# Tanveer81/ReVisionLLM

Hardware: AMD Instinct MI355X
Metric: video-segments/sec (whole node), stage-2 100-seg recursion, Vicuna-7B (higher is better)
Workload: dtype fp16

## Files before the change

### revisionllm_amd/csrc/gemm_rows.hip

```cpp
#include <hip/hip_runtime.h>

#include <atomic>
#include <type_traits>

#include "kernels.h"
#include "gemv_finish.h"

#ifndef RS_PROBE
#define RS_PROBE 0
#endif
#ifndef RS_PART
#define RS_PART 0
#endif
#ifndef RS_DW_BIG
#define RS_DW_BIG 4
#endif

namespace {

typedef const __attribute__((address_space(1))) void* gptr_t;
typedef __attribute__((address_space(3))) void* lptr_t;
__device__ __forceinline__ void glds16(const void* g, void* l) { __builtin_amdgcn_global_load_lds((gptr_t)g, (lptr_t)l, 16, 0, 0); }

typedef unsigned int rs_u32x4 __attribute__((ext_vector_type(4)));
constexpr int RS_SC1 = 16;
__device__ __forceinline__ void st_sc1(__amdgpu_buffer_rsrc_t r, unsigned byte_off, f32x4 v) {
    __builtin_amdgcn_raw_buffer_store_b128(__builtin_bit_cast(rs_u32x4, v), r, (int)byte_off, 0, RS_SC1);
}
__device__ __forceinline__ f32x4 ld_sc1(__amdgpu_buffer_rsrc_t r, unsigned byte_off) {
    return __builtin_bit_cast(f32x4, __builtin_amdgcn_raw_buffer_load_b128(r, (int)byte_off, 0, RS_SC1));
}

constexpr int RS_W = 4;
constexpr int RS_THREADS = (RS_W + 1) * 64;
template <int MB, int WP = 1> struct RowsCfg {
    static constexpr int DW = WP == 2 ? 8 : (MB >= 8 ? RS_DW_BIG : 4), LPS = WP == 2 ? 2 : 4, DX = MB == 4 ? 4 : 3, WPE = MB <= 5 ? 3 : 2;
};
typedef unsigned int rs_w8 __attribute__((ext_vector_type(4)));

constexpr bool rows_sumsq_at_head(int MB) { return MB >= 8; }
template <int MB, int NTH, int PTB>
__device__ __forceinline__ void rows_sumsq(const GemvNorm& nrm, float* ssq, int tg) {
    if (!nrm.in_sumsq || (RS_PROBE & 16)) return;
    constexpr int CHAINS = MB * 128;
    constexpr int PT = (CHAINS + NTH - 1) / NTH;
    const int nblk = nrm.in_nblk;
    const int off = (RS_PROBE & 2048) ? 0 : (int)((blockIdx.x >> 3) * 37u) % CHAINS;
#pragma unroll
    for (int i0 = 0; i0 < PT; i0 += PTB) {
        f32x4 pj[PTB][8];
        int cc[PTB];
#pragma unroll
        for (int i = 0; i < PTB; ++i) {
            const int idx = tg + (i0 + i) * NTH;
            int c = idx + off;
            c = c >= CHAINS ? c - CHAINS : c;
            cc[i] = (i0 + i < PT && idx < CHAINS) ? c : -1;
            const int mb = c >> 7, q = (c >> 2) & 31, rq = c & 3;
            const float* src = nrm.in_sumsq + ((int64_t)(mb * nblk + q) * 16 + rq * 4);
#pragma unroll
            for (int j = 0; j < 8; ++j) {
                const bool have = q + 32 * j < nblk;
                const f32x4 v = *(const f32x4*)(src + (have ? j * 512 : 0));
                pj[i][j] = have ? v : f32x4{0.f, 0.f, 0.f, 0.f};
            }
        }
        __builtin_amdgcn_sched_barrier(0);
#pragma unroll
        for (int i = 0; i < PTB; ++i) {
            if (cc[i] < 0) continue;
            const int c = cc[i], mb = c >> 7, q = (c >> 2) & 31, rq = c & 3;
            f32x4 a = f32x4{0.f, 0.f, 0.f, 0.f};
#pragma unroll
            for (int j = 0; j < 8; ++j) a += pj[i][j];
            for (int b = q + 256; b < nblk; b += 32) a += *(const f32x4*)(nrm.in_sumsq + ((int64_t)(mb * nblk + b) * 16 + rq * 4));
            *(f32x4*)(ssq + mb * 512 + q * 16 + rq * 4) = a;
        }
    }
}

template <int MB>
__device__ __forceinline__ void rows_sumsq_total(const float* ssq, float* totl, int t) {
    if (t < MB * 16) {
        const int mb = t >> 4, row = t & 15;
        float tot = 0.f;
#pragma unroll
        for (int q = 0; q < 32; ++q) tot += ssq[(mb * 32 + q) * 16 + row];
        totl[t] = tot;
    }
}

template <int MB, int PPW, int PAIRS, int WP>
__device__ __forceinline__ void rows_qkv_finish(const f32x4 (&sres)[PPW], int wave, int cg, int fr, int kg, int M, const GemvNorm& nrm, const QkvRope& qr,
                                                const float* totl) {
    const int D = qr.H * 128;
    const int n0 = cg * 64;
    const int sec = n0 >= 2 * D ? 2 : n0 >= D ? 1 : 0;
    const int hd0 = n0 - sec * D, head = hd0 >> 7;
    int posv[PPW];
    f32x4 cf[PPW], wsc[PPW];
#pragma unroll
    for (int i = 0; i < PPW; ++i) {
        const int p = wave + RS_W * i < PAIRS ? wave + RS_W * i : PAIRS - 1;
        const int tile = p / MB, mb = p % MB, b = mb * 16 + fr;
        const int pc = (hd0 & 127) + tile * 16 + kg * 4;
        const int bc = b < M ? b : M - 1;
        posv[i] = b < M ? qr.row_pos[bc] : -1;
        cf[i] = sec < 2 ? *(const f32x4*)(qr.cs + ((int64_t)bc * 64 + (pc >> 1)) * 2) : f32x4{0.f, 0.f, 0.f, 0.f};
        if constexpr (WP == 2) wsc[i] = *(const f32x4*)(nrm.w_scale + n0 + tile * 16 + kg * 4);
    }
    __builtin_amdgcn_sched_barrier(0);
#pragma unroll
    for (int i = 0; i < PPW; ++i) {
        const int p = wave + RS_W * i;
        if (p >= PAIRS) break;
        const int tile = p / MB, mb = p % MB, b = mb * 16 + fr;
        const int pc = (hd0 & 127) + tile * 16 + kg * 4;
        f32x4 v = sres[i];
        if constexpr (WP == 2) v *= wsc[i];
        if (nrm.in_sumsq) v *= rsqrtf(__fmaf_rn(totl[mb * 16 + fr], nrm.inv_d, nrm.eps));
        const int pos = posv[i];
        if (pos < 0 || pos >= qr.Smax) continue;
        if (sec < 2) {
            const f32x4 t = cf[i];
            const float a0 = __fmaf_rn(v[0], t[0], -__fmul_rn(v[1], t[1])), b0 = __fmaf_rn(v[1], t[0], __fmul_rn(v[0], t[1]));
            const float a1 = __fmaf_rn(v[2], t[2], -__fmul_rn(v[3], t[3])), b1 = __fmaf_rn(v[3], t[2], __fmul_rn(v[2], t[3]));
            const u32x2 o = pack_op16x4(f32x4{a0, b0, a1, b1});
            if (sec == 0) *(u32x2*)((op16_t*)qr.q16 + (int64_t)b * D + hd0 + tile * 16 + kg * 4) = o;
            else *(u32x2*)((op16_t*)qr.kc + (((int64_t)b * qr.H + head) * qr.Smax + pos) * 128 + pc) = o;
        } else {
            op16_t* dst = (op16_t*)qr.vtc + ((int64_t)b * qr.H + head) * 128 * qr.Smax + rv_vt_index(pc, pos);
#pragma unroll
            for (int r = 0; r < 4; ++r) dst[r * 8] = f32_to_op16(v[r]);
        }
    }
}

#ifndef RS_PF_N
#define RS_PF_N 8
#endif
constexpr int RS_PF = RS_PF_N;
#ifndef RS_EARLY_READS
#define RS_EARLY_READS 0
#endif
constexpr bool rows_early(int MB) { return RS_EARLY_READS && MB >= 8 && !(RS_PROBE & (4 | 4096)); }
template <int MB, int WP>
__device__ __forceinline__ void rows_stage_schedule() {
#ifndef RS_NO_STAGE_SCHEDULE
    if constexpr (MB >= 8 && !(RS_PROBE & 4)) {
        constexpr int R = 4 * MB;
        if constexpr (!rows_early(MB)) __builtin_amdgcn_sched_group_barrier(0x100, RS_PF, 0);
#ifdef RS_EARLY_PIN_VMEM
        else __builtin_amdgcn_sched_group_barrier(0x020, WP == 2 ? 2 : 4, 0);
#endif
#pragma unroll
        for (int i = 0; i < R - RS_PF; ++i) {
            __builtin_amdgcn_sched_group_barrier(0x008, 1, 0);
            __builtin_amdgcn_sched_group_barrier(0x100, 1, 0);
        }
        __builtin_amdgcn_sched_group_barrier(0x008, RS_PF, 0);
    }
#endif
}

template <int MB, int VPW, int FIN, int WP = 1>
__global__ __attribute__((amdgpu_flat_work_group_size(RS_THREADS, RS_THREADS), amdgpu_waves_per_eu(RowsCfg<MB>::WPE, RowsCfg<MB>::WPE))) void
rows_kernel(const op16_t* __restrict__ X, const op16_t* __restrict__ W, float* __restrict__ planes, const float* __restrict__ bias,
            const float* res, int64_t ldr, void* Cv, int64_t ldc, int M, int N, int K, GemvNorm nrm, QkvRope qr) {
    extern __shared__ __attribute__((aligned(16))) char rs_smem[];
    constexpr int S = 8 / VPW, LOG = VPW == 8 ? 3 : VPW == 4 ? 2 : VPW == 2 ? 1 : 0;
    constexpr int DW = RowsCfg<MB, WP>::DW, DX = RowsCfg<MB, WP>::DX, LPS = RowsCfg<MB, WP>::LPS;
    constexpr int SLAB = MB * 4096;
    constexpr int XL = MB * 4;
    static_assert((DX - 2) * XL <= 63 && (DW - 2) * LPS <= 63, "vmcnt is a 6-bit counter");
    const int tid = threadIdx.x, lane = tid & 63;
    const int wave = __builtin_amdgcn_readfirstlane(tid >> 6);
    const int cg = blockIdx.x / S, sp = blockIdx.x % S;
    const int nkb = K >> 7;
    const int ntile = cg * RS_W + (wave < RS_W ? wave : 0);
    auto vcount = [&](int i) -> int { return (nkb - (sp * VPW + i) + 7) >> 3; };
    int T = 0;
#pragma unroll
    for (int i = 0; i < VPW; ++i) T += vcount(i);

    f32x4 acc[MB], stk[LOG ? LOG : 1][MB];
#pragma unroll
    for (int mb = 0; mb < MB; ++mb) acc[mb] = f32x4{0.f, 0.f, 0.f, 0.f};

    if (wave == RS_W) {
        int pi = 0, pc = 0;
        auto next_kb = [&]() -> int {
            int kb = -1;
            if (pi < VPW) {
                kb = sp * VPW + pi + 8 * pc;
                if (++pc == vcount(pi)) { pc = 0; ++pi; }
            }
            return kb;
        };
        auto issue = [&](int g) {
            const int kb = next_kb();
            const op16_t* xs = X + (kb >= 0 ? (int64_t)kb * (MB * 2048) : 0) + lane * 8;
            char* dst = rs_smem + (g % DX) * SLAB;
#pragma unroll
            for (int i = 0; i < XL; ++i) glds16(xs + i * 512, dst + i * 1024);
        };
        if constexpr (!(RS_PROBE & 8))
            for (int d = 0; d < DX - 1; ++d) issue(d);
        if constexpr (rows_sumsq_at_head(MB)) {
            if (nrm.in_sumsq && !(RS_PROBE & 16)) __builtin_amdgcn_s_barrier();
        }
        for (int g = 0; g < T; ++g) {
            asm volatile("s_waitcnt vmcnt(%0)" ::"n"((DX - 2) * XL) : "memory");
            if constexpr (!(RS_PROBE & 2)) __builtin_amdgcn_s_barrier();
            if constexpr (!(RS_PROBE & 8)) issue(g + DX - 1);
        }
        asm volatile("s_waitcnt vmcnt(0)" ::: "memory");
    } else {
        const op16_t* wp = W + (int64_t)ntile * (K >> 5) * (WP == 2 ? 256 : 512) + lane * 8;
        typename std::conditional<WP == 2, rs_w8, op16x8>::type wf[DW][LPS];
        int li = 0, lc = 0;
        int ci = 0, cc = 0;
#define RS_ISSUE_W(slot)                                                                                                             \
    do {                                                                                                                             \
        int kb_ = -1;                                                                                                                \
        if (li < VPW) {                                                                                                              \
            kb_ = sp * VPW + li + 8 * lc;                                                                                            \
            if (++lc == vcount(li)) { lc = 0; ++li; }                                                                                \
        }                                                                                                                            \
        const op16_t* ws_ = kb_ >= 0 ? ((RS_PROBE & 1) ? W + lane * 8 + (kb_ & 1) * 2048 : wp + (int64_t)((RS_PROBE & 8192) ? (kb_ + ((int)blockIdx.x * RS_W + wave) * 5) % nkb : kb_) * (WP == 2 ? 1024 : 2048)) : X + lane * 8; \
        _Pragma("unroll") for (int j_ = 0; j_ < LPS; ++j_)                                                                          \
            wf[slot][j_] = __builtin_nontemporal_load((const typename std::remove_reference<decltype(wf[0][0])>::type*)(ws_ + j_ * 512)); \
    } while (0)
#pragma unroll
        for (int d = 0; d < DW - 1; ++d) RS_ISSUE_W(d);
        if constexpr (rows_sumsq_at_head(MB)) {
            if (nrm.in_sumsq && !(RS_PROBE & 16)) {
                float* ssq_ = (float*)(rs_smem + DX * SLAB);
                rows_sumsq<MB, 256, 3>(nrm, ssq_, tid);
                asm volatile("s_waitcnt lgkmcnt(0)" ::: "memory");
                __builtin_amdgcn_s_barrier();
                rows_sumsq_total<MB>(ssq_, ssq_ + MB * 512, tid);
                asm volatile("s_waitcnt lgkmcnt(0)" ::: "memory");
            }
        }
        unsigned long long* stamps = (unsigned long long*)(rs_smem + DX * SLAB + MB * (2048 + 64));
        const bool stamping = (RS_PROBE & 16384) && S == 1 && wave == 0 && blockIdx.x == 8;
#define RS_STAMP(k_)                                                                       \
    if constexpr (RS_PROBE & 16384) {                                                      \
        if (stamping && g < 64) {                                                          \
            const unsigned long long t_ = __builtin_amdgcn_s_memtime();                    \
            if (lane == 0) stamps[g * 4 + (k_)] = t_;                                      \
        }                                                                                  \
    }
        if constexpr (RS_PROBE & 16384) {
            if (stamping) {
                for (int i = lane; i < 256; i += 64) stamps[i] = 0ull;
            }
        }
        for (int g0 = 0; g0 < T; g0 += DW) {
#pragma unroll
            for (int u = 0; u < DW; ++u) {
                const int g = g0 + u;
                if (g < T) {
                    RS_STAMP(0)
                    asm volatile("s_waitcnt vmcnt(%0)" ::"n"((DW - 2) * LPS) : "memory");
                    RS_STAMP(1)
                    if constexpr (!(RS_PROBE & 2)) __builtin_amdgcn_s_barrier();
                    RS_STAMP(2)
                    op16x8 pre[rows_early(MB) ? RS_PF : 1];
                    if constexpr (rows_early(MB)) {
                        const char* xs0 = rs_smem + (g % DX) * SLAB + lane * 16;
#pragma unroll
                        for (int i = 0; i < RS_PF; ++i) pre[i] = *(const op16x8*)(xs0 + i * 1024);
                    }
                    RS_ISSUE_W((u + DW - 1) % DW);
                    {
                        const char* xs = rs_smem + (g % DX) * SLAB + lane * 16;
#pragma unroll
                        for (int j = 0; j < 4; ++j) {
                            op16x8 wj;
                            if constexpr (WP == 2) wj = fp8x8_to_op16x8(wf[u][j >> 1][(j & 1) * 2], wf[u][j >> 1][(j & 1) * 2 + 1]);
                            else wj = wf[u][j];
#pragma unroll
                            for (int mb = 0; mb < MB; ++mb) {
                                const op16x8 xf = (rows_early(MB) && j * MB + mb < RS_PF) ? pre[(j * MB + mb) % RS_PF]
                                                                                           : *(const op16x8*)(xs + ((RS_PROBE & 4096) ? 0 : (j * MB + mb) * 1024));
                                if constexpr (RS_PROBE & 4) {
                                    if (mb == 0) acc[0][0] += __builtin_bit_cast(f32x4, wj)[j & 3] + __builtin_bit_cast(f32x4, xf)[0];
                                } else {
                                    acc[mb] = rv_mfma16(wj, xf, acc[mb]);
                                }
                            }
                        }
                        rows_stage_schedule<MB, WP>();
                    }
                    RS_STAMP(3)
                    if (++cc == vcount(ci)) {
                        if constexpr (VPW > 1) {
                            bool placed = false;
#pragma unroll
                            for (int b = 0; b < LOG; ++b) {
                                if (placed) continue;
                                if ((ci >> b) & 1) {
#pragma unroll
                                    for (int mb = 0; mb < MB; ++mb) acc[mb] = stk[b][mb] + acc[mb];
                                } else {
#pragma unroll
                                    for (int mb = 0; mb < MB; ++mb) stk[b][mb] = acc[mb];
                                    placed = true;
                                }
                            }
                            if (placed) {
#pragma unroll
                                for (int mb = 0; mb < MB; ++mb) acc[mb] = f32x4{0.f, 0.f, 0.f, 0.f};
                            }
                        }
                        cc = 0;
                        ++ci;
                    }
                }
            }
        }
#undef RS_ISSUE_W
#undef RS_STAMP
        if constexpr (RS_PROBE & 16384) {
            if (stamping) {
                asm volatile("s_waitcnt lgkmcnt(0)" ::: "memory");
                for (int i = lane; i < 256; i += 64) ((unsigned long long*)planes)[i] = stamps[i];
            }
        }
    }
    const unsigned plane = (unsigned)(N >> 4) * MB * 1024;
    const __amdgpu_buffer_rsrc_t pr = __builtin_amdgcn_make_buffer_rsrc(planes, 0, 0x7ffffff0, 0x00020000);
    constexpr int XCH_OFF = MB * 2048 > 16384 ? MB * 2048 : 16384;
    static_assert(XCH_OFF + RS_W * MB * 1024 <= DX * MB * 4096, "the exchange area must fit the slab ring");
    char* xch = rs_smem + XCH_OFF;
    if constexpr (S == 1) {
        asm volatile("s_waitcnt vmcnt(0)" ::: "memory");
        __syncthreads();
        if (wave < RS_W) {
#pragma unroll
            for (int mb = 0; mb < MB; ++mb) *(f32x4*)(xch + ((wave * MB + mb) * 64 + lane) * 16) = acc[mb];
        }
    } else {
        if (wave < RS_W) {
            const unsigned off = sp * plane + ((unsigned)ntile * MB * 64 + lane) * 16;
#pragma unroll
            for (int mb = 0; mb < MB; ++mb) st_sc1(pr, off + mb * 1024, acc[mb]);
        }
        asm volatile("s_waitcnt vmcnt(0)" ::: "memory");
    }
    __syncthreads();
    __shared__ int is_last;
    if constexpr (S > 1) {
        if (tid == 0) {
            unsigned* cnt = (unsigned*)nrm.arrive + (LOG * (RV_ROWS_COUNTERS / 4) + cg);
            is_last = __hip_atomic_fetch_add(cnt, 1u, __ATOMIC_RELAXED, __HIP_MEMORY_SCOPE_AGENT) % S == S - 1;
        }
        __syncthreads();
        if (!is_last) return;
    }
    constexpr int NT = (FIN == 1 || FIN == 2) ? 2 : 1;
    constexpr int OUT_BF16 = (FIN == 1 || FIN == 4) ? 1 : 0;
    constexpr int ACT = FIN == 1 ? RV_ACT_SILU_MUL : RV_ACT_NONE;
    constexpr int ROPE = FIN == 3 ? 1 : 0;
    constexpr int BPG = RS_W / NT;
    constexpr int PAIRS = BPG * MB;
    constexpr int PPW = (PAIRS + RS_W - 1) / RS_W;
    const int fr = lane & 15, kg = lane >> 4;
    const int nblk = N / (16 * NT);
    f32x4 pl[PPW][NT][S];
    if (wave < RS_W) {
#pragma unroll
        for (int i = 0; i < PPW; ++i) {
            const int p = wave + RS_W * i < PAIRS ? wave + RS_W * i : PAIRS - 1;
            const int blk = cg * BPG + p / MB, mb = p % MB;
#pragma unroll
            for (int t = 0; t < NT; ++t) {
                if constexpr (S == 1) {
                    pl[i][t][0] = *(const f32x4*)(xch + (((p / MB * NT + t) * MB + mb) * 64 + lane) * 16);
                } else {
                    const unsigned q = (((unsigned)(blk * NT + t) * MB + mb) * 64 + lane) * 16;
#pragma unroll
                    for (int w = 0; w < S; ++w) pl[i][t][w] = ld_sc1(pr, q + w * plane);
                }
            }
        }
    }
    float* ssq = (float*)(rs_smem + (rows_sumsq_at_head(MB) ? DX * SLAB : 0));
    if constexpr (!rows_sumsq_at_head(MB)) {
        if (nrm.in_sumsq && !(RS_PROBE & 16)) {
            rows_sumsq<MB, RS_THREADS, 2>(nrm, ssq, tid);
            __syncthreads();
            rows_sumsq_total<MB>(ssq, ssq + MB * 512, tid);
            __syncthreads();
        }
    }
    const float* totl = ssq + MB * 512;
    if (wave >= RS_W) return;
    if constexpr (ROPE) {
        if (qr.row_pos && qr.G == 1 && !(RS_PROBE & 64)) {
            f32x4 sv[PPW];
#pragma unroll
            for (int i = 0; i < PPW; ++i) {
                if constexpr (S == 8) sv[i] = gemv_tree8(pl[i][0]);
                else if constexpr (S == 4) sv[i] = (pl[i][0][0] + pl[i][0][1]) + (pl[i][0][2] + pl[i][0][3]);
                else if constexpr (S == 2) sv[i] = pl[i][0][0] + pl[i][0][1];
                else sv[i] = pl[i][0][0];
            }
            rows_qkv_finish<MB, PPW, PAIRS, WP>(sv, wave, cg, fr, kg, M, nrm, qr, totl);
            return;
        }
    }
#pragma unroll
    for (int i = 0; i < PPW; ++i) {
        const int p = wave + RS_W * i;
        if (p >= PAIRS) break;
        const int blk = cg * BPG + p / MB, mb = p % MB;
        f32x4 sres[NT];
#pragma unroll
        for (int t = 0; t < NT; ++t) {
            if constexpr (S == 8) sres[t] = gemv_tree8(pl[i][t]);
            else if constexpr (S == 4) sres[t] = (pl[i][t][0] + pl[i][t][1]) + (pl[i][t][2] + pl[i][t][3]);
            else if constexpr (S == 2) sres[t] = pl[i][t][0] + pl[i][t][1];
            else sres[t] = pl[i][t][0];
        }
        const float tot = nrm.in_sumsq ? totl[mb * 16 + fr] : 0.f;
        const f32x4 z = f32x4{0.f, 0.f, 0.f, 0.f};
        gemv_finish<NT, OUT_BF16, ACT, WP, ROPE>(sres, mb, fr, kg, blk, nblk, M, N, bias, res, ldr, Cv, ldc, nrm, qr, tot, z, z, z, z, false);
    }
}

constexpr int RS_MAXIT = 8;
template <int MB, int VPW, int FIN, int WP = 1>
__global__ __attribute__((amdgpu_flat_work_group_size(RS_THREADS, RS_THREADS), amdgpu_waves_per_eu(RowsCfg<MB>::WPE, RowsCfg<MB>::WPE))) void
rows_kernel_p(const op16_t* __restrict__ X, const op16_t* __restrict__ W, float* __restrict__ planes, const float* __restrict__ bias,
            const float* res, int64_t ldr, void* Cv, int64_t ldc, int M, int N, int K, GemvNorm nrm, QkvRope qr) {
    extern __shared__ __attribute__((aligned(16))) char rs_smem[];
    constexpr int S = 8 / VPW, LOG = VPW == 8 ? 3 : VPW == 4 ? 2 : VPW == 2 ? 1 : 0;
    constexpr int DW = RowsCfg<MB, WP>::DW, DX = RowsCfg<MB, WP>::DX, LPS = RowsCfg<MB, WP>::LPS;
    constexpr int SLAB = MB * 4096;
    constexpr int XL = MB * 4;
    static_assert((DX - 2) * XL <= 63 && (DW - 2) * LPS <= 63, "vmcnt is a 6-bit counter");
    const int tid = threadIdx.x, lane = tid & 63;
    const int wave = __builtin_amdgcn_readfirstlane(tid >> 6);
    const int nitems = (N >> 6) * S, G = (int)gridDim.x;
    const int sp = blockIdx.x % S;
    const int nkb = K >> 7;
    const int n_it = (nitems - (int)blockIdx.x + G - 1) / G;
    auto vcount = [&](int i) -> int { return (nkb - (sp * VPW + i) + 7) >> 3; };
    int T = 0;
#pragma unroll
    for (int i = 0; i < VPW; ++i) T += vcount(i);
    const int Tp = (T + DW - 1) / DW * DW;
    const unsigned plane = (unsigned)(N >> 4) * MB * 1024;
    const __amdgpu_buffer_rsrc_t pr = __builtin_amdgcn_make_buffer_rsrc(planes, 0, 0x7ffffff0, 0x00020000);

    f32x4 acc[MB], stk[LOG ? LOG : 1][MB];
#pragma unroll
    for (int mb = 0; mb < MB; ++mb) acc[mb] = f32x4{0.f, 0.f, 0.f, 0.f};

    if (wave == RS_W) {
        int pi = 0, pc = 0, pp = 0, pn = 0;
        auto issue = [&](int g) {
            int kb = -1;
            if (pn < n_it) {
                if (pp < T) {
                    kb = sp * VPW + pi + 8 * pc;
                    if (++pc == vcount(pi)) { pc = 0; ++pi; }
                }
                if (++pp == Tp) { pp = 0; pi = 0; ++pn; }
            }
            const op16_t* xs = X + (kb >= 0 ? (int64_t)kb * (MB * 2048) : 0) + lane * 8;
            char* dst = rs_smem + (g % DX) * SLAB;
#pragma unroll
            for (int i = 0; i < XL; ++i) glds16(xs + i * 512, dst + i * 1024);
        };
        if constexpr (!(RS_PROBE & 8))
            for (int d = 0; d < DX - 1; ++d) issue(d);
        if constexpr (rows_sumsq_at_head(MB)) {
            if (nrm.in_sumsq && !(RS_PROBE & 16)) __builtin_amdgcn_s_barrier();
        }
        const int TT = n_it * Tp;
        for (int g = 0; g < TT; ++g) {
            asm volatile("s_waitcnt vmcnt(%0)" ::"n"((DX - 2) * XL) : "memory");
            if constexpr (!(RS_PROBE & 2)) __builtin_amdgcn_s_barrier();
            if constexpr (!(RS_PROBE & 8)) issue(g + DX - 1);
        }
    } else {
        const int64_t tile_stride = (int64_t)(K >> 5) * (WP == 2 ? 256 : 512);
        const int64_t item_stride = (int64_t)(G / S) * RS_W * tile_stride;
        const op16_t* wp = W + ((int)blockIdx.x / S * RS_W + wave) * tile_stride + lane * 8;
        typename std::conditional<WP == 2, rs_w8, op16x8>::type wf[DW][LPS];
        int li = 0, lc = 0, lp = 0, ln = 0;
#define RS_ISSUE_W(slot)                                                                                                             \
    do {                                                                                                                             \
        const op16_t* ws_ = X + lane * 8;                                                                                            \
        if (ln < n_it) {                                                                                                             \
            if (lp < T) {                                                                                                            \
                const int kb_ = sp * VPW + li + 8 * lc;                                                                              \
                ws_ = (RS_PROBE & 1) ? W + lane * 8 + (kb_ & 1) * 2048 : wp + (int64_t)((RS_PROBE & 8192) ? (kb_ + ((int)blockIdx.x * RS_W + wave) * 5) % (K >> 7) : kb_) * (WP == 2 ? 1024 : 2048);                 \
                if (++lc == vcount(li)) { lc = 0; ++li; }                                                                            \
            }                                                                                                                        \
            if (++lp == Tp) { lp = 0; li = 0; ++ln; wp += item_stride; }                                                             \
        }                                                                                                                            \
        _Pragma("unroll") for (int j_ = 0; j_ < LPS; ++j_)                                                                          \
            wf[slot][j_] = __builtin_nontemporal_load((const typename std::remove_reference<decltype(wf[0][0])>::type*)(ws_ + j_ * 512)); \
    } while (0)
#pragma unroll
        for (int d = 0; d < DW - 1; ++d) RS_ISSUE_W(d);
        if constexpr (rows_sumsq_at_head(MB)) {
            if (nrm.in_sumsq && !(RS_PROBE & 16)) {
                float* ssq_ = (float*)(rs_smem + DX * SLAB);
                rows_sumsq<MB, 256, 3>(nrm, ssq_, tid);
                asm volatile("s_waitcnt lgkmcnt(0)" ::: "memory");
                __builtin_amdgcn_s_barrier();
                rows_sumsq_total<MB>(ssq_, ssq_ + MB * 512, tid);
                asm volatile("s_waitcnt lgkmcnt(0)" ::: "memory");
            }
        }
        int g = 0;
        for (int n = 0; n < n_it; ++n) {
            int ci = 0, cc = 0;
            for (int s0 = 0; s0 < Tp; s0 += DW) {
#pragma unroll
                for (int u = 0; u < DW; ++u, ++g) {
                    asm volatile("s_waitcnt vmcnt(%0)" ::"n"((DW - 2) * LPS) : "memory");
                    if constexpr (!(RS_PROBE & 2)) __builtin_amdgcn_s_barrier();
                    op16x8 pre[rows_early(MB) ? RS_PF : 1];
                    if constexpr (rows_early(MB)) {
                        const char* xs0 = rs_smem + (g % DX) * SLAB + lane * 16;
#pragma unroll
                        for (int i = 0; i < RS_PF; ++i) pre[i] = *(const op16x8*)(xs0 + i * 1024);
                    }
                    RS_ISSUE_W((u + DW - 1) % DW);
                    if (s0 + u < T) {
                        const char* xs = rs_smem + (g % DX) * SLAB + lane * 16;
#pragma unroll
                        for (int j = 0; j < 4; ++j) {
                            op16x8 wj;
                            if constexpr (WP == 2) wj = fp8x8_to_op16x8(wf[u][j >> 1][(j & 1) * 2], wf[u][j >> 1][(j & 1) * 2 + 1]);
                            else wj = wf[u][j];
#pragma unroll
                            for (int mb = 0; mb < MB; ++mb) {
                                const op16x8 xf = (rows_early(MB) && j * MB + mb < RS_PF) ? pre[(j * MB + mb) % RS_PF]
                                                                                           : *(const op16x8*)(xs + ((RS_PROBE & 4096) ? 0 : (j * MB + mb) * 1024));
                                if constexpr (RS_PROBE & 4) {
                                    if (mb == 0) acc[0][0] += __builtin_bit_cast(f32x4, wj)[j & 3] + __builtin_bit_cast(f32x4, xf)[0];
                                } else {
                                    acc[mb] = rv_mfma16(wj, xf, acc[mb]);
                                }
                            }
                        }
                        rows_stage_schedule<MB, WP>();
                        if (++cc == vcount(ci)) {
                            if constexpr (VPW > 1) {
                                bool placed = false;
#pragma unroll
                                for (int b = 0; b < LOG; ++b) {
                                    if (placed) continue;
                                    if ((ci >> b) & 1) {
#pragma unroll
                                        for (int mb = 0; mb < MB; ++mb) acc[mb] = stk[b][mb] + acc[mb];
                                    } else {
#pragma unroll
                                        for (int mb = 0; mb < MB; ++mb) stk[b][mb] = acc[mb];
                                        placed = true;
                                    }
                                }
                                if (placed) {
#pragma unroll
                                    for (int mb = 0; mb < MB; ++mb) acc[mb] = f32x4{0.f, 0.f, 0.f, 0.f};
                                }
                            }
                            cc = 0;
                            ++ci;
                        }
                    }
                }
            }
            if constexpr (S > 1) {
                const unsigned ntile = (unsigned)(((int)blockIdx.x + n * G) / S * RS_W + wave);
                const unsigned off = sp * plane + (ntile * MB * 64 + lane) * 16;
#pragma unroll
                for (int mb = 0; mb < MB; ++mb) {
                    st_sc1(pr, off + mb * 1024, acc[mb]);
                    acc[mb] = f32x4{0.f, 0.f, 0.f, 0.f};
                }
            }
        }
#undef RS_ISSUE_W
    }
    constexpr int XCH_OFF = MB * 2048 > 16384 ? MB * 2048 : 16384;
    static_assert(XCH_OFF + RS_W * MB * 1024 <= DX * MB * 4096, "the exchange area must fit the slab ring");
    char* xch = rs_smem + XCH_OFF;
    asm volatile("s_waitcnt vmcnt(0)" ::: "memory");
    __syncthreads();
    if constexpr (S == 1) {
        if (wave < RS_W) {
#pragma unroll
            for (int mb = 0; mb < MB; ++mb) *(f32x4*)(xch + ((wave * MB + mb) * 64 + lane) * 16) = acc[mb];
        }
        __syncthreads();
    }
    __shared__ int is_last[RS_MAXIT];
    if constexpr (S > 1) {
        if (tid < n_it) {
            unsigned* cnt = (unsigned*)nrm.arrive + (LOG * (RV_ROWS_COUNTERS / 4) + ((int)blockIdx.x + tid * G) / S);
            is_last[tid] = __hip_atomic_fetch_add(cnt, 1u, __ATOMIC_RELAXED, __HIP_MEMORY_SCOPE_AGENT) % S == S - 1;
        }
        __syncthreads();
        bool any = false;
        for (int n = 0; n < n_it; ++n) any = any || is_last[n];
        if (!any) return;
    }
    constexpr int NT = (FIN == 1 || FIN == 2) ? 2 : 1;
    constexpr int OUT_BF16 = (FIN == 1 || FIN == 4) ? 1 : 0;
    constexpr int ACT = FIN == 1 ? RV_ACT_SILU_MUL : RV_ACT_NONE;
    constexpr int ROPE = FIN == 3 ? 1 : 0;
    constexpr int BPG = RS_W / NT;
    constexpr int PAIRS = BPG * MB;
    constexpr int PPW = (PAIRS + RS_W - 1) / RS_W;
    const int fr = lane & 15, kg = lane >> 4;
    const int nblk = N / (16 * NT);
    float* ssq = (float*)(rs_smem + (rows_sumsq_at_head(MB) ? DX * SLAB : 0));
    if constexpr (!rows_sumsq_at_head(MB)) {
        if (nrm.in_sumsq && !(RS_PROBE & 16)) {
            rows_sumsq<MB, RS_THREADS, 2>(nrm, ssq, tid);
            __syncthreads();
            rows_sumsq_total<MB>(ssq, ssq + MB * 512, tid);
            __syncthreads();
        }
    }
    const float* totl = ssq + MB * 512;
    if (wave >= RS_W) return;
    for (int n = 0; n < n_it; ++n) {
        if constexpr (S > 1) {
            if (!is_last[n]) continue;
        }
        const int cg = ((int)blockIdx.x + n * G) / S;
        f32x4 pl[PPW][NT][S];
        if (wave < RS_W) {
#pragma unroll
            for (int i = 0; i < PPW; ++i) {
                const int p = wave + RS_W * i < PAIRS ? wave + RS_W * i : PAIRS - 1;
                const int blk = cg * BPG + p / MB, mb = p % MB;
#pragma unroll
                for (int t = 0; t < NT; ++t) {
                    if constexpr (S == 1) {
                        pl[i][t][0] = *(const f32x4*)(xch + (((p / MB * NT + t) * MB + mb) * 64 + lane) * 16);
                    } else {
                        const unsigned q = (((unsigned)(blk * NT + t) * MB + mb) * 64 + lane) * 16;
#pragma unroll
                        for (int w = 0; w < S; ++w) pl[i][t][w] = ld_sc1(pr, q + w * plane);
                    }
                }
            }
        }
#pragma unroll
        for (int i = 0; i < PPW; ++i) {
            const int p = wave + RS_W * i;
            if (p >= PAIRS) break;
            const int blk = cg * BPG + p / MB, mb = p % MB;
            f32x4 sres[NT];
#pragma unroll
            for (int t = 0; t < NT; ++t) {
                if constexpr (S == 8) sres[t] = gemv_tree8(pl[i][t]);
                else if constexpr (S == 4) sres[t] = (pl[i][t][0] + pl[i][t][1]) + (pl[i][t][2] + pl[i][t][3]);
                else if constexpr (S == 2) sres[t] = pl[i][t][0] + pl[i][t][1];
                else sres[t] = pl[i][t][0];
            }
            const float tot = nrm.in_sumsq ? totl[mb * 16 + fr] : 0.f;
            const f32x4 z = f32x4{0.f, 0.f, 0.f, 0.f};
            gemv_finish<NT, OUT_BF16, ACT, WP, ROPE>(sres, mb, fr, kg, blk, nblk, M, N, bias, res, ldr, Cv, ldc, nrm, qr, tot, z, z, z, z, false);
        }
    }
}

int rows_num_cus(int dev) {
    static std::atomic<int> cus[64];
    int n = cus[dev & 63].load(std::memory_order_relaxed);
    if (n == 0) {
        if (hipDeviceGetAttribute(&n, hipDeviceAttributeMultiprocessorCount, dev) != hipSuccess || n <= 0) n = 256;
        cus[dev & 63].store(n, std::memory_order_relaxed);
    }
    return n;
}
int rows_slots(int MBp) {
    int dev = 0;
    (void)hipGetDevice(&dev);
    return (rows_num_cus(dev) & ~7) * (MBp <= 5 ? 2 : 1);
}

int rows_splits(int64_t N, int MBp) {
    const int64_t cg = N / 64;
    int s = MBp >= 5 ? 2 : 1;
    const int fill = rv_cur_opts().rows_fill;
    if (MBp >= 8 && rv_cur_opts().rows_single && cg <= rows_slots(MBp) && cg * 4 >= (int64_t)rows_slots(MBp) * 3) return 1;
    while (s < 8 && cg * s < fill) s *= 2;
    if (rv_cur_opts().rows_persistent) {
        const int64_t slots = rows_slots(MBp);
        auto longest = [&](int s_) { return (cg * s_ + slots - 1) / slots * (8 / s_); };
        if (cg * s > slots)
            for (int s2 = s * 2; s2 <= 8; s2 *= 2)
                if (longest(s2) * 5 <= longest(s) * 4) s = s2;
    }
    return s;
}

#define RS_KERNEL (PERS ? rows_kernel_p<MB, VPW, FIN, WP> : rows_kernel<MB, VPW, FIN, WP>)
template <int MB, int VPW, int FIN, int WP, int PERS>
int rows_launch(const op16_t* X, const op16_t* W, const float* bias, const float* res, int64_t ldr, void* C, int64_t ldc, int M, int N, int K,
                const GemvNorm& nrm, const QkvRope& qr, hipStream_t st) {
    size_t lds = (size_t)RowsCfg<MB, WP>::DX * MB * 4096 + (rows_sumsq_at_head(MB) ? (size_t)MB * (2048 + 64) : 0)
                 + ((RS_PROBE & 16384) ? 2048 : 0);
    const unsigned items = (unsigned)(N / 64 * (8 / VPW));
    unsigned grid = items;
    if constexpr (PERS) {
        const unsigned slots = (unsigned)rows_slots(MB);
        if (slots >= 8 && slots < items) grid = slots;
    }
    RV_CHECK_ARG(items <= (unsigned)RS_MAXIT * grid, "gemm_rows: %u items for %u workgroups", items, grid);
    constexpr size_t alone = 81 * 1024;
    const bool spread = MB <= 5 && (int)grid <= rv_cur_opts().rows_spread;
    if (spread && lds < alone) lds = alone;
    static std::atomic<uint64_t> opted{0};
    int dev = 0;
    (void)hipGetDevice(&dev);
    const uint64_t bit = 1ull << (dev & 63);
    if (lds > 65536 && !(opted.load(std::memory_order_relaxed) & bit)) {
        if (hipFuncSetAttribute((const void*)RS_KERNEL, hipFuncAttributeMaxDynamicSharedMemorySize,
                                (int)(MB <= 5 && lds < alone ? alone : lds)) != hipSuccess) {
            rv_set_error("gemm_rows: cannot reserve %zu bytes of LDS", lds);
            return RV_ERR_HIP;
        }
        opted.fetch_or(bit, std::memory_order_relaxed);
    }
    hipLaunchKernelGGL((RS_KERNEL), dim3(grid), dim3(RS_THREADS), lds, st, X, W, nrm.planes, bias, res, ldr, C,
                       ldc, M, N, K, nrm, qr);
    return RV_OK;
}
#undef RS_KERNEL
template <int MB, int FIN, int WP>
int rows_by_split(int S, const op16_t* X, const op16_t* W, const float* bias, const float* res, int64_t ldr, void* C, int64_t ldc, int M, int N, int K,
                  const GemvNorm& nrm, const QkvRope& qr, hipStream_t st) {
    const bool pers = S > 1 && rv_cur_opts().rows_persistent && (int64_t)(N / 64) * S > rows_slots(MB) && (MB != 5 || S == 4);
#define RS_LAUNCH(VPW_) (pers ? rows_launch<MB, VPW_, FIN, WP, 1>(X, W, bias, res, ldr, C, ldc, M, N, K, nrm, qr, st) \
                              : rows_launch<MB, VPW_, FIN, WP, 0>(X, W, bias, res, ldr, C, ldc, M, N, K, nrm, qr, st))
    switch (S) {
        case 1: return rows_launch<MB, 8, FIN, WP, 0>(X, W, bias, res, ldr, C, ldc, M, N, K, nrm, qr, st);
        case 2: return RS_LAUNCH(4);
        case 4: return RS_LAUNCH(2);
        default: return RS_LAUNCH(1);
    }
#undef RS_LAUNCH
}
template <int FIN, int WP>
int rows_by_mb(int MBp, int S, const op16_t* X, const op16_t* W, const float* bias, const float* res, int64_t ldr, void* C, int64_t ldc, int M, int N,
               int K, const GemvNorm& nrm, const QkvRope& qr, hipStream_t st) {
#if RS_PART & 2
    return MBp == 8 ? rows_by_split<8, FIN, WP>(S, X, W, bias, res, ldr, C, ldc, M, N, K, nrm, qr, st)
                    : rows_by_split<9, FIN, WP>(S, X, W, bias, res, ldr, C, ldc, M, N, K, nrm, qr, st);
#else
    return MBp == 4 ? rows_by_split<4, FIN, WP>(S, X, W, bias, res, ldr, C, ldc, M, N, K, nrm, qr, st)
                    : rows_by_split<5, FIN, WP>(S, X, W, bias, res, ldr, C, ldc, M, N, K, nrm, qr, st);
#endif
}
template <int WP>
int rows_by_fin(int MBp, int S, const op16_t* X, const op16_t* W, const float* bias, const float* res, int64_t ldr, void* C, int64_t ldc, int out_dtype,
                int act, int M, int N, int K, const GemvNorm& nrm, const QkvRope* qr, hipStream_t st) {
    const QkvRope q0{};
    if (qr) return rows_by_mb<3, WP>(MBp, S, X, W, nullptr, nullptr, 0, nullptr, 0, M, N, K, nrm, *qr, st);
    if (act == RV_ACT_SILU_MUL) return rows_by_mb<1, WP>(MBp, S, X, W, bias, res, ldr, C, ldc, M, N, K, nrm, q0, st);
    if (N >= 16384 && out_dtype == RV_F32) return rows_by_mb<2, WP>(MBp, S, X, W, bias, res, ldr, C, ldc, M, N, K, nrm, q0, st);
    if (N < 16384 && out_dtype == RV_OP16) return rows_by_mb<4, WP>(MBp, S, X, W, bias, res, ldr, C, ldc, M, N, K, nrm, q0, st);
    if (N < 16384) return rows_by_mb<0, WP>(MBp, S, X, W, bias, res, ldr, C, ldc, M, N, K, nrm, q0, st);
    rv_set_error("gemm_rows: bf16 output with N >= 16384 is not instantiated");
    return RV_ERR_ARG;
}

}

#define RS_PART_FN_(n) gemm_rows_part##n
#define RS_PART_FN(n) RS_PART_FN_(n)
int RS_PART_FN(RS_PART)(int MBp, int S, const op16_t* X, const op16_t* W, const float* bias, const float* res, int64_t ldr, void* C, int64_t ldc,
                        int out_dtype, int act, int M, int N, int K, const GemvNorm& nrm, const QkvRope* qr, hipStream_t st) {
    return rows_by_fin<(RS_PART & 1) ? 2 : 1>(MBp, S, X, W, bias, res, ldr, C, ldc, out_dtype, act, M, N, K, nrm, qr, st);
}

#if RS_PART == 0
#define RS_PART_DECL(n)                                                                                                                      \
    int gemm_rows_part##n(int MBp, int S, const op16_t* X, const op16_t* W, const float* bias, const float* res, int64_t ldr, void* C, int64_t ldc, \
                          int out_dtype, int act, int M, int N, int K, const GemvNorm& nrm, const QkvRope* qr, hipStream_t st)
RS_PART_DECL(1);
RS_PART_DECL(2);
RS_PART_DECL(3);

size_t gemm_rows_ws_bytes() { return (size_t)(2 * 32768 / 16) * RV_XP_MAX_BLOCKS * 1024; }
extern "C" size_t rv_gemm_rows_ws_bytes(void) { return gemm_rows_ws_bytes(); }

int gemm_rows(const op16_t* X, const op16_t* W, const float* bias, const float* res, int64_t ldr, void* C, int64_t ldc, int out_dtype, int act,
              int M, int N, int K, hipStream_t st, const GemvNorm& nrm, const QkvRope* qr, int w_layout) {
    RV_CHECK_ARG(w_layout == 1 || (w_layout == 2 && nrm.w_scale), "gemm_rows: bf16 (1) or fp8 + per-row scales (2) fragment-packed weights");
    RV_CHECK_ARG(M > 32 && M <= RV_ROWS_MAX && nrm.x_packed == rv_xp_blocks(M) && nrm.planes && nrm.arrive,
                 "gemm_rows: 33 .. 144 fragment-packed rows, a plane workspace and arrival counters");
    RV_CHECK_ARG(N / 64 <= RV_ROWS_COUNTERS / 4, "gemm_rows: too many column groups");
    RV_CHECK_ARG(N % 64 == 0 && K % 128 == 0 && K >= 1024 && N <= 32768, "gemm_rows: N %% 64, K %% 128, K >= 1024, N <= 32768");
    RV_CHECK_ARG(act == RV_ACT_NONE || act == RV_ACT_SILU_MUL, "gemm_rows: no activation or SILU_MUL");
    RV_CHECK_ARG(act != RV_ACT_SILU_MUL || out_dtype == RV_OP16, "gemm_rows: SILU_MUL writes bf16");
    const int MBp = nrm.x_packed, S = rows_splits(N, MBp);
    RV_CHECK_ARG((size_t)S * (N / 16) * MBp * 1024 <= gemm_rows_ws_bytes(), "gemm_rows: %d partial planes of N = %d do not fit the plane workspace", S, N);
    auto* part = MBp >= 8 ? (w_layout == 2 ? gemm_rows_part3 : gemm_rows_part2) : (w_layout == 2 ? gemm_rows_part1 : gemm_rows_part0);
    const int rc = part(MBp, S, X, W, bias, res, ldr, C, ldc, out_dtype, act, M, N, K, nrm, qr, st);
    if (rc) return rc;
    RV_CHECK_LAUNCH("gemm_rows");
    return RV_OK;
}

extern "C" int rv_gemm_rows(const void* Xp, const void* Wp, const float* w_scale, void* C, int32_t M, int32_t N, int32_t K, void* planes,
                            int32_t* arrive, int act, int out_dtype, void* stream) {
    RV_CHECK_ARG(Xp && Wp && C && planes && arrive, "rv_gemm_rows: null argument");
    GemvNorm nrm;
    nrm.w_scale = w_scale;
    nrm.x_packed = rv_xp_blocks(M);
    nrm.planes = (float*)planes;
    nrm.arrive = arrive;
    const int ldc = act == RV_ACT_SILU_MUL ? N / 2 : N;
    return gemm_rows((const op16_t*)Xp, (const op16_t*)Wp, nullptr, nullptr, 0, C, ldc, out_dtype, act, M, N, K, (hipStream_t)stream, nrm, nullptr,
                     w_scale ? 2 : 1);
}
#endif
```

Measured before the change: 6431.

## Add paired fixed-K stage loop for large row-block GEMM kernels

Adds a specialised main loop for the rows GEMM kernels (plain and persistent) when K is 4096, MB>=8, VPW>=2 and the weight ring holds 4 stages. The loop is fully unrolled into two groups of four stages that accumulate into two register sets and are folded with a fixed binary-tree pattern, replacing the generic per-stage stack bookkeeping and branches. The goal is to remove dynamic control flow and stack-placement logic from the inner loop so the compiler can schedule MFMAs and loads better. In exchange it uses more accumulator registers, which may raise register pressure, and the summation order changes slightly.

After: 6469 (median of 4 runs). No clear change (+0.6%).

```diff
diff --git a/revisionllm_amd/csrc/gemm_rows.hip b/revisionllm_amd/csrc/gemm_rows.hip
--- a/revisionllm_amd/csrc/gemm_rows.hip
+++ b/revisionllm_amd/csrc/gemm_rows.hip
@@ -163,7 +163,58 @@
 #endif
 }
 
-template <int MB, int VPW, int FIN, int WP = 1>
+template <int MB, int VPW, int WP, int DW> constexpr bool rows_paired() {
+    return MB >= 8 && VPW >= 2 && WP == 1 && DW == 4 && (RS_PROBE & ~16384) == 0 && !RS_EARLY_READS;
+}
+template <int MB, bool FIRST, typename WF>
+__device__ __forceinline__ void rows_pair_stage(const WF (&w)[4], const char* xs, f32x4 (&a)[MB]) {
+#pragma unroll
+    for (int j = 0; j < 4; ++j) {
+#pragma unroll
+        for (int mb = 0; mb < MB; ++mb) {
+            const op16x8 xf = *(const op16x8*)(xs + (j * MB + mb) * 1024);
+            if constexpr (FIRST) {
+                if (j == 0) {
+                    a[mb] = rv_mfma16(w[0], xf, f32x4{0.f, 0.f, 0.f, 0.f});
+                    continue;
+                }
+            }
+            a[mb] = rv_mfma16(w[j], xf, a[mb]);
+        }
+    }
+}
+template <int MB, int VPW, int LOGN>
+__device__ __forceinline__ void rows_pair_fold(int p, const f32x4 (&va)[MB], const f32x4 (&vb)[MB], f32x4 (&stk)[LOGN][MB]) {
+    if constexpr (VPW >= 4) {
+        if (p & 1) {
+            if constexpr (VPW == 8) {
+                if (p & 2) {
+#pragma unroll
+                    for (int mb = 0; mb < MB; ++mb) stk[2][mb] = stk[2][mb] + (stk[1][mb] + (va[mb] + vb[mb]));
+                } else {
+#pragma unroll
+                    for (int mb = 0; mb < MB; ++mb) stk[2][mb] = stk[1][mb] + (va[mb] + vb[mb]);
+                }
+            } else {
+#pragma unroll
+                for (int mb = 0; mb < MB; ++mb) stk[1][mb] = stk[1][mb] + (va[mb] + vb[mb]);
+            }
+        } else {
+#pragma unroll
+            for (int mb = 0; mb < MB; ++mb) stk[1][mb] = va[mb] + vb[mb];
+        }
+    }
+}
+template <int MB, int VPW, int LOGN>
+__device__ __forceinline__ void rows_pair_result(const f32x4 (&va)[MB], const f32x4 (&vb)[MB], const f32x4 (&stk)[LOGN][MB], f32x4 (&acc)[MB]) {
+#pragma unroll
+    for (int mb = 0; mb < MB; ++mb) {
+        if constexpr (VPW == 2) acc[mb] = va[mb] + vb[mb];
+        else acc[mb] = stk[LOGN - 1][mb];
+    }
+}
+
+template <int MB, int VPW, int FIN, int WP = 1, int PR = 0>
 __global__ __attribute__((amdgpu_flat_work_group_size(RS_THREADS, RS_THREADS), amdgpu_waves_per_eu(RowsCfg<MB>::WPE, RowsCfg<MB>::WPE))) void
 rows_kernel(const op16_t* __restrict__ X, const op16_t* __restrict__ W, float* __restrict__ planes, const float* __restrict__ bias,
             const float* res, int64_t ldr, void* Cv, int64_t ldc, int M, int N, int K, GemvNorm nrm, QkvRope qr) {
@@ -257,6 +308,37 @@
                 for (int i = lane; i < 256; i += 64) stamps[i] = 0ull;
             }
         }
+#define RS_PSTAGE(ACC_, G_, U_, FIRST_)                                                                                              \
+    {                                                                                                                                \
+        const int g = (G_);                                                                                                          \
+        RS_STAMP(0)                                                                                                                  \
+        asm volatile("s_waitcnt vmcnt(%0)" ::"n"((DW - 2) * LPS) : "memory");                                                        \
+        RS_STAMP(1)                                                                                                                  \
+        __builtin_amdgcn_s_barrier();                                                                                                \
+        RS_STAMP(2)                                                                                                                  \
+        RS_ISSUE_W(((U_) + DW - 1) % DW);                                                                                            \
+        rows_pair_stage<MB, FIRST_>(wf[U_], rs_smem + (g % DX) * SLAB + lane * 16, ACC_);                                            \
+        rows_stage_schedule<MB, WP>();                                                                                               \
+        RS_STAMP(3)                                                                                                                  \
+    }
+        if constexpr (PR) {
+            {
+                static_assert(!PR || rows_paired<MB, VPW, WP, DW>(), "the paired loop: 8 / 9 row blocks, bf16 / fp16 weights, a ring of 4");
+                f32x4 va[MB], vb[MB];
+                for (int p = 0; p < VPW / 2; ++p) {
+                    RS_PSTAGE(va, p * 8 + 0, 0, true)
+                    RS_PSTAGE(va, p * 8 + 1, 1, false)
+                    RS_PSTAGE(va, p * 8 + 2, 2, false)
+                    RS_PSTAGE(va, p * 8 + 3, 3, false)
+                    RS_PSTAGE(vb, p * 8 + 4, 0, true)
+                    RS_PSTAGE(vb, p * 8 + 5, 1, false)
+                    RS_PSTAGE(vb, p * 8 + 6, 2, false)
+                    RS_PSTAGE(vb, p * 8 + 7, 3, false)
+                    rows_pair_fold<MB, VPW>(p, va, vb, stk);
+                }
+                rows_pair_result<MB, VPW>(va, vb, stk, acc);
+            }
+        } else
         for (int g0 = 0; g0 < T; g0 += DW) {
 #pragma unroll
             for (int u = 0; u < DW; ++u) {
@@ -321,6 +403,7 @@
                 }
             }
         }
+#undef RS_PSTAGE
 #undef RS_ISSUE_W
 #undef RS_STAMP
         if constexpr (RS_PROBE & 16384) {
@@ -432,7 +515,7 @@
 }
 
 constexpr int RS_MAXIT = 8;
-template <int MB, int VPW, int FIN, int WP = 1>
+template <int MB, int VPW, int FIN, int WP = 1, int PR = 0>
 __global__ __attribute__((amdgpu_flat_work_group_size(RS_THREADS, RS_THREADS), amdgpu_waves_per_eu(RowsCfg<MB>::WPE, RowsCfg<MB>::WPE))) void
 rows_kernel_p(const op16_t* __restrict__ X, const op16_t* __restrict__ W, float* __restrict__ planes, const float* __restrict__ bias,
             const float* res, int64_t ldr, void* Cv, int64_t ldc, int M, int N, int K, GemvNorm nrm, QkvRope qr) {
@@ -520,6 +603,45 @@
             }
         }
         int g = 0;
+#define RS_STORE_ITEM(n_)                                                                                                            \
+    if constexpr (S > 1) {                                                                                                           \
+        const unsigned ntile = (unsigned)(((int)blockIdx.x + (n_) * G) / S * RS_W + wave);                                           \
+        const unsigned off = sp * plane + (ntile * MB * 64 + lane) * 16;                                                             \
+        _Pragma("unroll") for (int mb = 0; mb < MB; ++mb) {                                                                          \
+            st_sc1(pr, off + mb * 1024, acc[mb]);                                                                                    \
+            acc[mb] = f32x4{0.f, 0.f, 0.f, 0.f};                                                                                     \
+        }                                                                                                                            \
+    }
+#define RS_PSTAGE(ACC_, U_, FIRST_)                                                                                                  \
+    {                                                                                                                                \
+        asm volatile("s_waitcnt vmcnt(%0)" ::"n"((DW - 2) * LPS) : "memory");                                                        \
+        __builtin_amdgcn_s_barrier();                                                                                                \
+        RS_ISSUE_W(((U_) + DW - 1) % DW);                                                                                            \
+        rows_pair_stage<MB, FIRST_>(wf[U_], rs_smem + (g % DX) * SLAB + lane * 16, ACC_);                                            \
+        rows_stage_schedule<MB, WP>();                                                                                               \
+        ++g;                                                                                                                         \
+    }
+        if constexpr (PR) {
+            {
+                static_assert(!PR || rows_paired<MB, VPW, WP, DW>(), "the paired loop: 8 / 9 row blocks, bf16 / fp16 weights, a ring of 4");
+                f32x4 va[MB], vb[MB];
+                for (int n = 0; n < n_it; ++n) {
+                    for (int p = 0; p < VPW / 2; ++p) {
+                        RS_PSTAGE(va, 0, true)
+                        RS_PSTAGE(va, 1, false)
+                        RS_PSTAGE(va, 2, false)
+                        RS_PSTAGE(va, 3, false)
+                        RS_PSTAGE(vb, 0, true)
+                        RS_PSTAGE(vb, 1, false)
+                        RS_PSTAGE(vb, 2, false)
+                        RS_PSTAGE(vb, 3, false)
+                        rows_pair_fold<MB, VPW>(p, va, vb, stk);
+                    }
+                    rows_pair_result<MB, VPW>(va, vb, stk, acc);
+                    RS_STORE_ITEM(n)
+                }
+            }
+        } else
         for (int n = 0; n < n_it; ++n) {
             int ci = 0, cc = 0;
             for (int s0 = 0; s0 < Tp; s0 += DW) {
@@ -579,16 +701,10 @@
                     }
                 }
             }
-            if constexpr (S > 1) {
-                const unsigned ntile = (unsigned)(((int)blockIdx.x + n * G) / S * RS_W + wave);
-                const unsigned off = sp * plane + (ntile * MB * 64 + lane) * 16;
-#pragma unroll
-                for (int mb = 0; mb < MB; ++mb) {
-                    st_sc1(pr, off + mb * 1024, acc[mb]);
-                    acc[mb] = f32x4{0.f, 0.f, 0.f, 0.f};
-                }
-            }
-        }
+            RS_STORE_ITEM(n)
+        }
+#undef RS_PSTAGE
+#undef RS_STORE_ITEM
 #undef RS_ISSUE_W
     }
     constexpr int XCH_OFF = MB * 2048 > 16384 ? MB * 2048 : 16384;
@@ -708,9 +824,9 @@
     return s;
 }
 
-#define RS_KERNEL (PERS ? rows_kernel_p<MB, VPW, FIN, WP> : rows_kernel<MB, VPW, FIN, WP>)
-template <int MB, int VPW, int FIN, int WP, int PERS>
-int rows_launch(const op16_t* X, const op16_t* W, const float* bias, const float* res, int64_t ldr, void* C, int64_t ldc, int M, int N, int K,
+#define RS_KERNEL (PERS ? rows_kernel_p<MB, VPW, FIN, WP, PR> : rows_kernel<MB, VPW, FIN, WP, PR>)
+template <int MB, int VPW, int FIN, int WP, int PERS, int PR>
+int rows_launch_pr(const op16_t* X, const op16_t* W, const float* bias, const float* res, int64_t ldr, void* C, int64_t ldc, int M, int N, int K,
                 const GemvNorm& nrm, const QkvRope& qr, hipStream_t st) {
     size_t lds = (size_t)RowsCfg<MB, WP>::DX * MB * 4096 + (rows_sumsq_at_head(MB) ? (size_t)MB * (2048 + 64) : 0)
                  + ((RS_PROBE & 16384) ? 2048 : 0);
@@ -741,6 +857,14 @@
     return RV_OK;
 }
 #undef RS_KERNEL
+template <int MB, int VPW, int FIN, int WP, int PERS>
+int rows_launch(const op16_t* X, const op16_t* W, const float* bias, const float* res, int64_t ldr, void* C, int64_t ldc, int M, int N, int K,
+                const GemvNorm& nrm, const QkvRope& qr, hipStream_t st) {
+    if constexpr (rows_paired<MB, VPW, WP, RowsCfg<MB, WP>::DW>()) {
+        if (K == 4096) return rows_launch_pr<MB, VPW, FIN, WP, PERS, 1>(X, W, bias, res, ldr, C, ldc, M, N, K, nrm, qr, st);
+    }
+    return rows_launch_pr<MB, VPW, FIN, WP, PERS, 0>(X, W, bias, res, ldr, C, ldc, M, N, K, nrm, qr, st);
+}
 template <int MB, int FIN, int WP>
 int rows_by_split(int S, const op16_t* X, const op16_t* W, const float* bias, const float* res, int64_t ldr, void* C, int64_t ldc, int M, int N, int K,
                   const GemvNorm& nrm, const QkvRope& qr, hipStream_t st) {
```
